# DJNing/articulated-object-nerf

Measured on AMD Instinct MI355X. Metric: rays/sec at 640×480×(64c+128f) samples; PSNR vs reference, higher is better.
Workload: dtype f16x3 (fp16 hi/lo split MFMA, fp32 accumulate)

## Files before the change

articulated-object-nerf_amd/aonerf/_lib.py:

```python
import ctypes
import os

import torch

_HERE = os.path.dirname(os.path.abspath(__file__))
LIB_PATH = os.path.join(os.path.dirname(_HERE), "lib", "libaonerf.so")

c_i64, c_int, c_float, c_size, vp = ctypes.c_int64, ctypes.c_int, ctypes.c_float, ctypes.c_size_t, ctypes.c_void_p

PREC = {"fp32": 0, "f16x3": 1}
PREC_F16X3_TRAIN = 1
PREC_BF16 = 2
ACT_NONE, ACT_VANILLA, ACT_ARTIC = 0, 1, 2
OPACITY = {None: 0, "mse": 1, "ce": 2, "autorf": 3}


class AonMlpParams(ctypes.Structure):
    _fields_ = [("pts_w", vp * 8), ("pts_b", vp * 8), ("density_w", vp), ("density_b", vp),
                ("bottleneck_w", vp), ("bottleneck_b", vp), ("views_w", vp), ("views_b", vp),
                ("rgb_w", vp), ("rgb_b", vp), ("w_rows", c_i64 * 12), ("w_cols", c_i64 * 12),
                ("b_len", c_i64 * 12)]


class AonMlpArtParams(ctypes.Structure):
    _fields_ = [("def_w", vp * 4), ("def_b", vp * 4), ("deformation_w", vp), ("deformation_b", vp),
                ("pts_w", vp * 8), ("pts_b", vp * 8), ("density_w", vp), ("density_b", vp),
# ... 336 lines not shown
```

articulated-object-nerf_amd/csrc/mlp.hip:

```cpp
#include "aon_common.hpp"
#include "mlp_layout.hpp"
#include "mlp_pipe.hpp"
#include "param_check.hpp"

namespace aon {
namespace mlp {

constexpr int kWaves = 8;
constexpr int kThreads = 64 * kWaves;
constexpr int kRowsPerWave = 16;
constexpr int kRowsPerBlock = kRowsPerWave * kWaves;

__device__ __forceinline__ f4 mfma(float a, float b, f4 c) {
  return __builtin_amdgcn_mfma_f32_16x16x4f32(a, b, c, 0, 0, 0);
}

template <int LAYER, int NA, int NB, int NACC>
__device__ __forceinline__ void gemm(Pipe<kThreads>& p, const f4 (&xa)[NA], const f4 (&xb)[NB],
                                     f4 (&acc)[NACC]) {
  constexpr LayerDesc d = kLayers[LAYER];
  constexpr int U = d.u;
  static_assert(U % 4 == 0 && U <= NACC && d.ka <= NA && d.kb <= NB, "layer/array mismatch");
#pragma unroll
  for (int t = 0; t < d.ka + d.kb; ++t) {
// ... 191 lines not shown
      while (li + 1 < kNumLayers && a.layers[li + 1].bias0 <= i) ++li;
      const int o = i - a.layers[li].bias0;
      if (o < a.layers[li].out_real) v = a.b[li][o];
    }
    out[e] = v;
  }
}

}
}

using namespace aon;
using namespace aon::mlp;

extern "C" size_t aon_mlp_packed_bytes(int precision) {
  if (precision == AON_PREC_FP32 || precision == AON_PREC_F16X3 || precision == AON_PREC_BF16)
    return kPackedBytesF32;
  return 0;
}

extern "C" int aon_mlp_read_status(const void* packed, size_t packed_bytes, uint32_t* status,
                                   aon_stream_t stream) {
  AON_REQUIRE(packed && status, "null pointer");
  AON_REQUIRE(packed_bytes >= kStatusBytes && packed_bytes % 16 == 0, "bad packed size");
  const char* word = static_cast<const char*>(packed) + packed_bytes - kStatusBytes;
  hipError_t e = hipMemcpyAsync(status, word, sizeof(uint32_t), hipMemcpyDeviceToHost,
                                (hipStream_t)stream);
  if (e == hipSuccess) e = hipStreamSynchronize((hipStream_t)stream);
  return static_cast<int>(e);
}

#ifndef AON_F16X3_NCOL
#define AON_F16X3_NCOL 1
#endif
static_assert(AON_F16X3_NCOL == 1 || AON_F16X3_NCOL == 2, "AON_F16X3_NCOL is 1 or 2");

extern "C" int aon_mlp_pack(const aon_mlp_params* prm, int precision, void* packed,
                            aon_stream_t stream) {
  AON_REQUIRE(prm && packed, "null pointer");
  AON_REQUIRE(precision == AON_PREC_FP32 || precision == AON_PREC_F16X3 ||
                  precision == AON_PREC_BF16,
              "unsupported precision");
  AON_REQUIRE(aligned16(packed), "packed buffer must be 16-byte aligned");
  if (check_mlp_params(prm, __func__)) return -1;
  PackArgs a;
  for (int i = 0; i < 8; ++i) {
    a.w[i] = prm->pts_w[i];
    a.b[i] = prm->pts_b[i];
  }
  a.w[LDEN] = prm->density_w;    a.b[LDEN] = prm->density_b;
  a.w[LBOT] = prm->bottleneck_w; a.b[LBOT] = prm->bottleneck_b;
  a.w[LVIEW] = prm->views_w;     a.b[LVIEW] = prm->views_b;
  a.w[LRGB] = prm->rgb_w;        a.b[LRGB] = prm->rgb_b;
  for (int i = 0; i < kNumLayers; ++i) {
    AON_REQUIRE(a.w[i] && a.b[i], "null layer parameter");
    a.layers[i] = precision == AON_PREC_FP32 ? kLayers[i] : kLayersH[i];
  }
  if (precision != AON_PREC_FP32)
    return pack_f16x3(a, packed, (hipStream_t)stream, precision == AON_PREC_BF16);
  const hipError_t e = hipMemsetAsync(static_cast<char*>(packed) + kPackedBytesF32 - kStatusBytes, 0,
                                      kStatusBytes, (hipStream_t)stream);
  if (e != hipSuccess) return static_cast<int>(e);
  const int64_t total = (int64_t)kStreamBlocks * 256 + kBiasFloats;
  hipLaunchKernelGGL(k_pack_f32, grid_for(total, 256, 4096), 256, 0, (hipStream_t)stream, a,
                     static_cast<float*>(packed));
  return launch_status(__func__);
}

static int mlp_launch(int mode, const void* packed, int precision, const float* a0,
                      const float* a1, const float* a2, const float* a3, int64_t B, int S,
                      int act, float* raw, aon_stream_t stream) {
  AON_REQUIRE(packed && raw && a0 && a1, "null pointer");
  AON_REQUIRE(precision == AON_PREC_FP32 || precision == AON_PREC_F16X3,
              "unsupported precision (AON_PREC_BF16 is the training forward's: aon_mlp_fwd_train_bf16)");
  AON_REQUIRE(B >= 0 && S >= 1, "bad shape");
  AON_REQUIRE(act >= AON_ACT_NONE && act <= AON_ACT_ARTIC, "bad activation");
  AON_REQUIRE(aligned16(packed) && aligned16(raw), "packed / raw must be 16-byte aligned");
  const int64_t N = B * S;
  if (N == 0) return 0;
  AON_REQUIRE((N + kRowsPerBlock - 1) / kRowsPerBlock < (1ll << 31), "too many rows");
#if AON_DATAFLOW_WS_BUILD
  if (precision == AON_PREC_F16X3 && mode == 0)
    return launch_ws_f16x3(packed, a0, a1, a2, a3, B, S, act, raw, (hipStream_t)stream);
#endif
  if (precision == AON_PREC_F16X3)
    return launch_f16x3(mode, AON_F16X3_NCOL, packed, a0, a1, a2, a3, B, S, act, raw,
                        (hipStream_t)stream);
// ... 64 lines not shown
```

articulated-object-nerf_amd/csrc/mlp_f16x3.hip:

```cpp
#include "mlp_f16x3_core.hpp"

namespace aon {
namespace mlp {

#ifndef AON_STASH_REGS
#define AON_STASH_REGS 0
#endif

#ifndef AON_STAGGER
#define AON_STAGGER 0
#endif

template <bool BF>
__host__ __device__ constexpr int stash_per() { return BF ? 3 : 6; }
template <bool BF>
__device__ __forceinline__ int enc_slot(int c, int k, int lo) { return BF ? 3 * c + k : 6 * c + 2 * k + lo; }
template <bool BF>
__device__ __forceinline__ int venc_slot(int c, int lo) { return BF ? 3 * c + 2 : 6 * c + 4 + lo; }

template <int NCOL, bool STORE, typename T, typename FP>
__device__ __forceinline__ void vanilla_layers(FP& fp, Frag<2, NCOL>& enc, Frag<1, NCOL>& venc,
                                               Frag<8, NCOL>& x, Frag<8, NCOL>& y, f4* stash,
                                               float* bias_s, int g, int wave,
                                               const int64_t (&rows)[NCOL], int64_t N, int act,
                                               float* __restrict__ raw, const TrainStore& ts) {
  constexpr bool BF = std::is_same<T, __bf16>::value;
  fp.start();
#if AON_PRIO_HALF
  if (wave >= GeomH<NCOL>::kWaves / 2) __builtin_amdgcn_s_setprio(AON_PRIO_HALF);
#endif
  lds_float* bias_l = opaque_lds(bias_s + 4 * g);

  Frag<1, NCOL> none;
  using SP = StorePick<STORE, NCOL, T>;
  T* const th = reinterpret_cast<T*>(ts.h);
  T* const tbot = reinterpret_cast<T*>(ts.bot);
  T* const thv = reinterpret_cast<T*>(ts.hv);
  const int64_t hs = act_rows(N) * 256;
  const int64_t ms = act_rows(N) * 4;
  layer_h<NetVanillaH, L0, true>(fp, none, enc, x, bias_l, g, SP::make(th, 256, rows, N, g, ts.masks));
  layer_h<NetVanillaH, L1, true>(fp, x, none, y, bias_l, g, SP::make(th + 1 * hs, 256, rows, N, g, ts.masks + 1 * ms));
  layer_h<NetVanillaH, L2, true>(fp, y, none, x, bias_l, g, SP::make(th + 2 * hs, 256, rows, N, g, ts.masks + 2 * ms));
  layer_h<NetVanillaH, L3, true>(fp, x, none, y, bias_l, g, SP::make(th + 3 * hs, 256, rows, N, g, ts.masks + 3 * ms));
  layer_h<NetVanillaH, L4, true>(fp, y, none, x, bias_l, g, SP::make(th + 4 * hs, 256, rows, N, g, ts.masks + 4 * ms));
#pragma unroll
  for (int c = 0; c < NCOL && !AON_STASH_REGS; ++c)
#pragma unroll
    for (int k = 0; k < 2; ++k) {
      enc.hi[k][c] = __builtin_bit_cast(h8, stash[64 * enc_slot<BF>(c, k, 0)]);
      if (!BF) enc.lo[k][c] = __builtin_bit_cast(h8, stash[64 * enc_slot<BF>(c, k, 1)]);
    }
  layer_h<NetVanillaH, L5, true>(fp, x, enc, y, bias_l, g, SP::make(th + 5 * hs, 256, rows, N, g, ts.masks + 5 * ms));
  layer_h<NetVanillaH, L6, true>(fp, y, none, x, bias_l, g, SP::make(th + 6 * hs, 256, rows, N, g, ts.masks + 6 * ms));
  layer_h<NetVanillaH, L7, true>(fp, x, none, y, bias_l, g, SP::make(th + 7 * hs, 256, rows, N, g, ts.masks + 7 * ms));
  f4 dens[NCOL], rgb[NCOL];
  head_h<NetVanillaH, LDEN>(fp, y, dens, bias_l, g);
  layer_h<NetVanillaH, LBOT, false>(fp, y, none, x, bias_l, g, SP::make(tbot, 256, rows, N, g));
#pragma unroll
  for (int c = 0; c < NCOL && !AON_STASH_REGS; ++c) {
    venc.hi[0][c] = __builtin_bit_cast(h8, stash[64 * venc_slot<BF>(c, 0)]);
    if (!BF) venc.lo[0][c] = __builtin_bit_cast(h8, stash[64 * venc_slot<BF>(c, 1)]);
  }
  layer_h<NetVanillaH, LVIEW, true>(fp, x, venc, y, bias_l, g, SP::make(thv, 128, rows, N, g, ts.masks + 8 * ms));
  head_h<NetVanillaH, LRGB>(fp, y, rgb, bias_l, g);

  if (g == 0) {
#pragma unroll
    for (int c = 0; c < NCOL; ++c) {
      if (rows[c] < N) {
        const float s = AON_F16X3_V2 ? 1.0f : 1.0f / kActScale;
        float sig = dens[c][0] * s;
        if (STORE && ts.noise) sig = __fadd_rn(sig, ts.noise[rows[c]]);
        const f4 o = {act_rgb(rgb[c][0] * s, act), act_rgb(rgb[c][1] * s, act),
                      act_rgb(rgb[c][2] * s, act), act_sigma(sig, act)};
#ifdef AON_ABL_NO_RAW_STORE
        if (__builtin_isnan(o[0] + o[1] + o[2] + o[3]))
#endif
        *reinterpret_cast<f4*>(raw + 4 * rows[c]) = o;
      }
    }
  }
}

template <int MODE, int NCOL, bool STORE = false, bool BF = false>
__global__ __launch_bounds__((GeomH<NCOL, BF>::kThreads), (GeomH<NCOL, BF>::kWavesPerSimd)) void k_mlp_fwd_f16x3(
    const f4* __restrict__ wstream, const float* __restrict__ bias_g, const float* __restrict__ in0,
    const float* __restrict__ in1, const float* __restrict__ in2, const float* __restrict__ in3,
    int64_t B, int S, int act, float* __restrict__ raw, TrainStore ts = {}) {
  using G = GeomH<NCOL, BF>;
  constexpr int kPer = stash_per<BF>() * NCOL;
  constexpr int kStash = AON_STASH_REGS ? 0 : G::kWaves * 64 * kPer;
  static_assert((kLdsWeights + kBiasFloats / 4 + kStash) * 16 <= 160 * 1024, "LDS");
  __shared__ f4 smem[kLdsWeights + kBiasFloats / 4 + kStash];
  float* bias_s = reinterpret_cast<float*>(smem + kLdsWeights);
  f4* stash = smem + kLdsWeights + kBiasFloats / 4 + (threadIdx.x >> 6) * 64 * kPer +
              (threadIdx.x & 63);

  const int tid = threadIdx.x, lane = tid & 63, wave = tid >> 6;
  const int g = lane >> 4, j = lane & 15;
  const int64_t N = B * S;

  WeightPipeP<NetVanillaH, G::kThreads, BF> p;
  p.wbuf = smem;
  p.src = wstream;
  p.tid = tid;
  p.lane = lane;
  p.start();
  for (int i = tid; i < kBiasFloats; i += G::kThreads) bias_s[i] = bias_g[i];

  Frag<2, NCOL> enc;
  Frag<1, NCOL> venc;
  int64_t rows[NCOL];
#pragma unroll
  for (int c = 0; c < NCOL; ++c) {
    const int64_t row = (int64_t)blockIdx.x * G::kRowsPerBlock + wave * G::kRowsPerWave + 16 * c + j;
    rows[c] = row;
    const int64_t rr = row < N ? row : N - 1;
    const int64_t ray = rr / S;
    float ev[2][8], vv[8];
    if (MODE == 0) {
      const float* ro = in0 + 3 * ray;
      const float* rd = in1 + 3 * ray;
      const float* vd = in2 + 3 * ray;
// ... 49 lines not shown
    split8<BF>(vv, venc.hi[0][c], venc.lo[0][c], venc.ovf);
  }

#pragma unroll
  for (int c = 0; c < NCOL && !AON_STASH_REGS; ++c) {
#pragma unroll
    for (int k = 0; k < 2; ++k) {
      stash[64 * enc_slot<BF>(c, k, 0)] = __builtin_bit_cast(f4, enc.hi[k][c]);
      if (!BF) stash[64 * enc_slot<BF>(c, k, 1)] = __builtin_bit_cast(f4, enc.lo[k][c]);
    }
    stash[64 * venc_slot<BF>(c, 0)] = __builtin_bit_cast(f4, venc.hi[0][c]);
    if (!BF) stash[64 * venc_slot<BF>(c, 1)] = __builtin_bit_cast(f4, venc.lo[0][c]);
  }

  Frag<8, NCOL> x, y;
  using WP = WeightPipeP<NetVanillaH, G::kThreads, BF>;
  using T = typename std::conditional<BF, __bf16, float>::type;
  if (AON_STAGGER && NCOL == 1 && !STORE && __builtin_amdgcn_readfirstlane(wave) >= G::kWaves / 2) {
    FragPipe<WP, AON_PREFETCH, 4, BF> fp(p);
    vanilla_layers<NCOL, STORE, T>(fp, enc, venc, x, y, stash, bias_s, g, wave, rows, N, act, raw, ts);
  } else {
    FragPipe<WP, AON_PREFETCH, 0, BF> fp(p);
    vanilla_layers<NCOL, STORE, T>(fp, enc, venc, x, y, stash, bias_s, g, wave, rows, N, act, raw, ts);
  }
  range_report(bias_g + kBiasFloats, ovf_of(x) | ovf_of(y) | enc.ovf | venc.ovf);
}

__global__ void k_pack_h(PackArgsH a, float* __restrict__ out_f) {
  const int64_t nhalf = (int64_t)a.stream_blocks * 512;
  _Float16* out = reinterpret_cast<_Float16*>(out_f);
  float* bias_out = out_f + (int64_t)a.stream_blocks * 256;
  const int64_t total = nhalf + a.bias_floats;
  const LayerDesc& last = a.layers[a.n_layers - 1];
  const int used_blocks = last.blk0 + (last.ka + last.kb) * last.u * 2;
  const StreamMap map{a.bf16, a.mx_lo, a.mx_hi};
  if (a.bf16 == 1 && !a.f16w && blockIdx.x == 0 && threadIdx.x < kStatusBytes / 4)
    reinterpret_cast<uint32_t*>(bias_out + a.bias_floats)[threadIdx.x] = 0u;
  for (int64_t e = blockIdx.x * (int64_t)blockDim.x + threadIdx.x; e < total;
       e += (int64_t)gridDim.x * blockDim.x) {
    if (e < nhalf) {
// ... 20 lines not shown
        const int o = 16 * u + (l & 15), gg = l >> 4;
        int col = -1;
        const float* src = a.w[li];
        int64_t ld = a.ldw[li];
        if (k < d.ka) {
          const int f = 32 * k + 16 * (jj >> 2) + 4 * gg + (jj & 3);
          col = f < d.len_a ? f : -1;
        } else {
          const int f = 32 * (k - d.ka) + 8 * gg + jj;
          col = f < d.len_b ? (a.w2[li] ? f : d.len_a + f) : -1;
          if (a.w2[li]) {
            src = a.w2[li];
            ld = a.ldw2[li];
          }
        }
        if (o < d.out_real && col >= 0)
          w = a.tr[li] ? src[(int64_t)col * ld + o] : src[(int64_t)o * ld + col];
      }
#if AON_F16X3_V2
      if (bf && !a.f16w) {
        out[e] = bf_bits(w);
        continue;
      }
      w *= kWS;
      const _Float16 h = static_cast<_Float16>(w);
      out[e] = lo_part ? static_cast<_Float16>(w - static_cast<float>(h)) : h;
      if (!lo_part && !(fabsf(w) <= kF16Max))
        *reinterpret_cast<uint32_t*>(bias_out + a.bias_floats) = 2u;
#else
      const _Float16 h = static_cast<_Float16>(w);
      out[e] = lo_part ? static_cast<_Float16>((w - static_cast<float>(h)) * kLoScale) : h;
#endif
    } else {
      const int i = static_cast<int>(e - nhalf);
      int li = 0;
      while (li + 1 < a.n_layers && a.layers[li + 1].bias0 <= i) ++li;
      const int o = i - a.layers[li].bias0;
#if AON_F16X3_V2
      const StreamMap map{a.bf16, a.mx_lo, a.mx_hi};
      const float bs =
          a.layers[li].u == 1 || !(map.f16(a.layers[li].blk0) || a.f16w) ? 1.0f : kActS;
#else
      const float bs = kActScale;
#endif
      bias_out[i] = (o < a.layers[li].out_real && a.b[li]) ? a.b[li][o] * bs : 0.f;
    }
  }
}

int pack_h(PackArgsH a, void* packed, hipStream_t stream) {
  const int64_t total = (int64_t)a.stream_blocks * 512 + a.bias_floats;
  if (a.bf16 != 1 || a.f16w) {
    const hipError_t e = hipMemsetAsync(
        static_cast<char*>(packed) + (size_t)a.stream_blocks * 1024 + (size_t)a.bias_floats * 4, 0,
        kStatusBytes, stream);
    if (e != hipSuccess) return static_cast<int>(e);
  }
  hipLaunchKernelGGL(k_pack_h, grid_for(total, 256, 4096), 256, 0, stream, a,
                     static_cast<float*>(packed));
  return launch_status("aon_mlp_pack");
}

int pack_f16x3(const PackArgs& a, void* packed, hipStream_t stream, bool bf16) {
  PackArgsH h{};
  h.bf16 = bf16 ? 1 : 0;
  for (int i = 0; i < kNumLayers; ++i) {
    h.w[i] = a.w[i];
    h.b[i] = a.b[i];
    h.layers[i] = kLayersH[i];
    h.ldw[i] = kLayersH[i].len_a + kLayersH[i].len_b;
  }
  h.n_layers = kNumLayers;
  h.stream_blocks = NetVanillaH::kStreamBlocks;
  h.bias_floats = NetVanillaH::kBiasFloats;
  return pack_h(h, packed, stream);
}

int launch_f16x3(int mode, int ncol, const void* packed, const float* a0, const float* a1,
                 const float* a2, const float* a3, int64_t B, int S, int act, float* raw,
                 hipStream_t stream, const TrainStore* ts) {
  const int64_t N = B * S;
  const f4* ws = static_cast<const f4*>(packed);
  const float* bias = reinterpret_cast<const float*>(static_cast<const char*>(packed) + kStreamBytesF32);
#define AON_LAUNCH_H(M, C)                                                                       \
  hipLaunchKernelGGL((k_mlp_fwd_f16x3<M, C>),                                                    \
                     static_cast<int>((N + GeomH<C>::kRowsPerBlock - 1) / GeomH<C>::kRowsPerBlock), \
                     GeomH<C>::kThreads, 0, stream, ws, bias, a0, a1, a2, a3, B, S, act, raw)
  if (mode == 2 || mode == 3) {
    const int grid = static_cast<int>((N + GeomH<1>::kRowsPerBlock - 1) / GeomH<1>::kRowsPerBlock);
    if (mode == 3) {
      using GB = GeomH<kBfNcolFwd, true>;
      hipLaunchKernelGGL((k_mlp_fwd_f16x3<0, kBfNcolFwd, true, true>),
                         static_cast<int>((N + GB::kRowsPerBlock - 1) / GB::kRowsPerBlock),
                         GB::kThreads, 0, stream, ws, bias, a0, a1, a2, a3, B, S, act, raw, *ts);
    } else
      hipLaunchKernelGGL((k_mlp_fwd_f16x3<0, 1, true>), grid, GeomH<1>::kThreads, 0, stream, ws,
                         bias, a0, a1, a2, a3, B, S, act, raw, *ts);
    return launch_status("aon_mlp_fwd_train");
  }
  if (mode == 0 && ncol == 1) AON_LAUNCH_H(0, 1);
  else if (mode == 0) AON_LAUNCH_H(0, 2);
  else if (ncol == 1) AON_LAUNCH_H(1, 1);
  else AON_LAUNCH_H(1, 2);
// ... 7 lines not shown
```

articulated-object-nerf_amd/csrc/mlp_layout.hpp:

```cpp
#pragma once

namespace aon {
namespace mlp {

struct LayerDesc {
  int ka, kb;
  int u;
  int len_a, len_b;
  int out_real;
  int blk0;
  int bias0;
};

enum { L0 = 0, L1, L2, L3, L4, L5, L6, L7, LDEN, LBOT, LVIEW, LRGB, kNumLayers };

constexpr int kChunk = 16;

constexpr LayerDesc kLayers[kNumLayers] = {
    {4, 0, 16, 63, 0, 256, 0, 0},
    {16, 0, 16, 256, 0, 256, 64, 256},
    {16, 0, 16, 256, 0, 256, 320, 512},
    {16, 0, 16, 256, 0, 256, 576, 768},
    {16, 0, 16, 256, 0, 256, 832, 1024},
    {16, 4, 16, 256, 63, 256, 1088, 1280},
// ... 7 lines not shown

constexpr LayerDesc kLayersH[kNumLayers] = {
    {0, 2, 16, 0, 63, 256, 0, 0},
    {8, 0, 16, 256, 0, 256, 64, 256},
    {8, 0, 16, 256, 0, 256, 320, 512},
    {8, 0, 16, 256, 0, 256, 576, 768},
    {8, 0, 16, 256, 0, 256, 832, 1024},
    {8, 2, 16, 256, 63, 256, 1088, 1280},
    {8, 0, 16, 256, 0, 256, 1408, 1536},
    {8, 0, 16, 256, 0, 256, 1664, 1792},
    {8, 0, 1, 256, 0, 1, 1920, 2048},
    {8, 0, 16, 256, 0, 256, 1936, 2064},
    {8, 1, 8, 256, 27, 128, 2192, 2320},
    {4, 0, 1, 128, 0, 3, 2336, 2448},
};

constexpr float kActScale = 1.0f / 256.0f;
constexpr float kLoScale = 2048.0f;
#ifndef AON_F16X3_V2
#define AON_F16X3_V2 1
#endif
constexpr float kActS = 8.0f;
constexpr float kWS = 64.0f;

constexpr int kBlocks = 2344;
constexpr int kStreamBlocks = (kBlocks + 63) / 64 * 64;
constexpr int kNumChunks = kStreamBlocks / kChunk;
constexpr int kBiasFloats = 2464;
constexpr size_t kStreamBytesF32 = (size_t)kStreamBlocks * 1024;
constexpr size_t kStatusBytes = 16;
// ... 111 lines not shown
    int blk = 0, bias = 0;
    for (int i = 0; i < NLAYERS; ++i) {
      const LayerDesc d = TABLE[i];
      if (d.blk0 != blk || d.bias0 != bias || d.blk0 % 2) return false;
      if (!(d.u == 1 || d.u % 2 == 0)) return false;
      if (d.len_a > 32 * d.ka || d.len_b > 32 * d.kb || d.out_real > 16 * d.u) return false;
      blk += (d.ka + d.kb) * d.u * 2;
      bias += d.u * 16;
    }
    return blk == BLOCKS && bias == BIAS_FLOATS && STREAM_BLOCKS >= BLOCKS &&
           STREAM_BLOCKS % 64 == 0;
  }
};

using NetVanillaH = NetH<kLayersH, kNumLayers, kBlocks, kStreamBlocks, kBiasFloats>;
using NetArtH = NetH<kLayersArt, kNumLayersArt, 2752, 2752, 3376>;
using NetBwdH = NetH<kLayersBwd, kNumLayersBwd, 2224, 2240, 2432, true>;
using NetArtBwdH = NetH<kLayersArtBwd, kNumLayersArtBwd, 2752, 2752, 3456, true>;
static_assert(NetVanillaH::ok(), "inconsistent vanilla fp16x3 layout");
static_assert(NetArtH::ok(), "inconsistent articulated fp16x3 layout");
static_assert(NetBwdH::ok(), "inconsistent backward-chain fp16x3 layout");
static_assert(NetArtBwdH::ok(), "inconsistent articulated backward-chain fp16x3 layout");

struct PackArgs {
  const float* w[kNumLayers];
  const float* b[kNumLayers];
  LayerDesc layers[kNumLayers];
};

constexpr int kMaxLayersH = 24;
struct PackArgsH {
  const float* w[kMaxLayersH];
  const float* w2[kMaxLayersH];
  const float* b[kMaxLayersH];
  int ldw[kMaxLayersH];
  int ldw2[kMaxLayersH];
  int tr[kMaxLayersH];
  LayerDesc layers[kMaxLayersH];
  int n_layers, stream_blocks, bias_floats;
  int bf16;
  int mx_lo, mx_hi;
  int f16w;
};

struct StreamMap {
  int mode, lo, hi;
  __host__ __device__ constexpr bool f16(int b) const {
    return mode == 0 || (mode == 2 && b >= lo && b < hi);
  }
  __host__ __device__ constexpr int map(int b) const {
    return mode == 0 ? b
         : mode == 1 ? b >> 1
         : b < lo    ? b >> 1
         : b < hi    ? (lo >> 1) + b - lo
                     : (lo >> 1) + (hi - lo) + ((b - hi) >> 1);
  }
  __host__ __device__ constexpr int unmap(int m) const {
// ... 32 lines not shown
  __bf16* enc_bf;
};

struct TrainStoreArt {
  float* hd;
  float* h;
  float* bot;
  float* hv;
  float* enc;
  float* xyz;
  const float* noise;
  uint2* masks;
  __bf16* enc_bf;
};

int pack_f16x3(const PackArgs& a, void* packed, hipStream_t stream, bool bf16 = false);
int pack_h(PackArgsH a, void* packed, hipStream_t stream);
int absmax(const float* x, int64_t n, uint32_t* out, hipStream_t stream);
int launch_f16x3(int mode, int ncol, const void* packed, const float* a0, const float* a1,
                 const float* a2, const float* a3, int64_t B, int S, int act, float* raw,
                 hipStream_t stream, const TrainStore* ts = nullptr);
#ifndef AON_DATAFLOW_WS_BUILD
#define AON_DATAFLOW_WS_BUILD 0
#endif
int launch_ws_f16x3(const void* packed, const float* a0, const float* a1, const float* a2,
                    const float* a3, int64_t B, int S, int act, float* raw, hipStream_t stream);
int launch_art_ws_f16x3(const void* packed, const float* a0, const float* a1, const float* a2,
                        const float* a3, int64_t B, int S, int act, float* raw, hipStream_t stream);

}
}
// ... 1 lines not shown
```

articulated-object-nerf_amd/csrc/mlp_ws.hip:

```cpp
#include <utility>

#include "mlp_f16x3_core.hpp"

namespace aon {
namespace mlp {
namespace ws {

#ifndef AON_WS_PREFETCH
#define AON_WS_PREFETCH 3
#endif

template <int WAVES>
struct Geo {
  static constexpr int kWaves = WAVES;
  static constexpr int kThreads = 64 * WAVES;
  static constexpr int kTiles = WAVES;
  static constexpr int kNb = 16 * kTiles;
  static constexpr int kActPlane = 8 * 4 * kNb;
  static constexpr int kEncPlane = 2 * 4 * kNb;
  static constexpr int kLdsF4 = 2 * kActPlane + 2 * kEncPlane;
  static constexpr int kWavesPerSimd = 2;
  static constexpr int kPrefetch = WAVES == 8 ? AON_WS_PREFETCH : AON_WS_PREFETCH - 1;
  static_assert(kLdsF4 * 16 * (8 / WAVES) <= 160 * 1024, "LDS");
  __host__ __device__ static constexpr int tu(int u) { return u / 2 >= WAVES ? u / WAVES : 2; }
// ... 244 lines not shown
  c.pl.act_hi = lds_base(smem + gj);
  c.pl.act_lo = lds_base(smem + G::kActPlane + gj);
  c.pl.enc_hi = lds_base(smem + 2 * G::kActPlane + gj);
  c.pl.enc_lo = lds_base(smem + 2 * G::kActPlane + G::kEncPlane + gj);
  c.row = (int64_t)blockIdx.x * G::kNb + 16 * c.w + c.j;
  c.rr = c.row < N ? c.row : N - 1;
  c.ray = c.rr / S;
  return c;
}

template <int WAVES>
__global__ __launch_bounds__(64 * WAVES, 2) void k_mlp_ws_f16x3(
    const f4* __restrict__ wstream, const float* __restrict__ bias_g, const float* __restrict__ in0,
    const float* __restrict__ in1, const float* __restrict__ in2, const float* __restrict__ in3,
    int64_t B, int S, int act, float* __restrict__ raw) {
  using Net = NetVanillaH;
  using G = Geo<WAVES>;
  __shared__ f4 smem[G::kLdsF4];
  const int64_t N = B * S;
  const WsSetup c = ws_setup<G>(smem, N, S);
  const int w = c.w, g = c.g;
  const Planes& pl = c.pl;
  APipe<Net, G, G::kPrefetch> ap;
  ap.ws = wstream;
  ap.lane = c.lane;
  ap.w = w;
  ap.start();

  uint64_t ovf = 0;
  {
    const float* ro = in0 + 3 * c.ray;
// ... 16 lines not shown
  hidden_layer<Net, G, L0, true>(ap, pl, bias_g, w, g, m16);
  hidden_layer<Net, G, L1, true>(ap, pl, bias_g, w, g, m16);
  hidden_layer<Net, G, L2, true>(ap, pl, bias_g, w, g, m16);
  hidden_layer<Net, G, L3, true>(ap, pl, bias_g, w, g, m16);
  hidden_layer<Net, G, L4, true>(ap, pl, bias_g, w, g, m16);
  hidden_layer<Net, G, L5, true>(ap, pl, bias_g, w, g, m16, [&] {
    const float* vd = in2 + 3 * c.ray;
    float vv[8];
#pragma unroll
    for (int e = 0; e < 8; ++e) vv[e] = pos_enc_feature(vd[0], vd[1], vd[2], 8 * g + e, 0, 4);
    put_segb<G>(pl, 0, w, vv, ovf);
  });
  hidden_layer<Net, G, L6, true>(ap, pl, bias_g, w, g, m16);
  hidden_layer<Net, G, L7, true>(ap, pl, bias_g, w, g, m16);
  const f4 dens = head<Net, G, LDEN>(ap, pl, bias_g, w, g);
  hidden_layer<Net, G, LBOT, false>(ap, pl, bias_g, w, g, m16);
  hidden_layer<Net, G, LVIEW, true>(ap, pl, bias_g, w, g, m16);
  const f4 rgb = head<Net, G, LRGB>(ap, pl, bias_g, w, g);
  if (g == 0 && c.row < N) {
    const f4 o = {act_rgb(rgb[0], act), act_rgb(rgb[1], act), act_rgb(rgb[2], act), act_sigma(dens[0], act)};
    *reinterpret_cast<f4*>(raw + 4 * c.row) = o;
  }
  const bool bad = (m16 & 0x7FFFu) >= 0x7C00u || ((m16 >> 16) & 0x7FFFu) >= 0x7C00u;
  range_report(bias_g + Net::kBiasFloats, ovf | __builtin_amdgcn_ballot_w64(bad));
}

template <int WAVES>
__global__ __launch_bounds__(64 * WAVES, 2) void k_mlp_art_ws_f16x3(
    const f4* __restrict__ wstream, const float* __restrict__ bias_g, const float* __restrict__ in0,
    const float* __restrict__ in1, const float* __restrict__ in2, const float* __restrict__ in3,
    int64_t B, int S, int act, float* __restrict__ raw) {
  using Net = NetArtH;
  using G = Geo<WAVES>;
// ... 311 lines not shown
#define AON_WS_HALVES(L_, RELU_, PREV, OUT)                                                  \
  f4 OUT##_a0[LG<Net, G, L_>::TU][LG<Net, G, L_>::NTh];                                     \
  half_mfma<Net, G, L_, 0>(ap, pl, w, OUT##_a0, PREV, m16);                                  \
  lds_barrier();                                                                             \
  const auto OUT##_j0 = make_job<Net, G, L_, RELU_, 0>(OUT##_a0, bias_g, w, g);              \
  f4 OUT##_a1[LG<Net, G, L_>::TU][LG<Net, G, L_>::NTh];                                     \
  half_mfma<Net, G, L_, 1>(ap, pl, w, OUT##_a1, OUT##_j0, m16);                              \
  lds_barrier();                                                                             \
  const auto OUT = make_job<Net, G, L_, RELU_, 1>(OUT##_a1, bias_g, w, g);

template <int WAVES>
__global__ __launch_bounds__(64 * WAVES, 2) void k_mlp_ws_pipe_f16x3(
    const f4* __restrict__ wstream, const float* __restrict__ bias_g, const float* __restrict__ in0,
    const float* __restrict__ in1, const float* __restrict__ in2, const float* __restrict__ in3,
    int64_t B, int S, int act, float* __restrict__ raw) {
  using Net = NetVanillaH;
  using G = Geo<WAVES>;
  __shared__ f4 smem[G::kLdsF4];
  const int64_t N = B * S;
  const WsSetup c = ws_setup<G>(smem, N, S);
  const int w = c.w, g = c.g;
  const Planes& pl = c.pl;
  APipeP<Net, G, G::kPrefetch> ap;
  ap.ws = wstream;
  ap.lane = c.lane;
  ap.w = w;
  ap.start();
  const bool first_half = w < G::kTiles / 2;

  uint64_t ovf = 0;
  {
// ... 20 lines not shown
  AON_WS_HALVES(L2, true, j1, j2)
  AON_WS_HALVES(L3, true, j2, j3)
  AON_WS_HALVES(L4, true, j3, j4)
  AON_WS_HALVES(L5, true, j4, j5)
  {
    const float* vd = in2 + 3 * c.ray;
    float vv[8];
#pragma unroll
    for (int e = 0; e < 8; ++e) vv[e] = pos_enc_feature(vd[0], vd[1], vd[2], 8 * g + e, 0, 4);
    put_segb<G>(pl, 0, w, vv, ovf);
  }
  AON_WS_HALVES(L6, true, j5, j6)
  AON_WS_HALVES(L7, true, j6, j7)
  f4 dens = {0.f, 0.f, 0.f, 0.f};
  if (first_half) dens = head_direct<Net, G, LDEN>(pl, wstream, bias_g, w, g, c.lane);
  f4 jb_a0[LG<Net, G, LBOT>::TU][LG<Net, G, LBOT>::NTh];
  half_mfma<Net, G, LBOT, 0>(ap, pl, w, jb_a0, j7, m16);
  lds_barrier();
  const auto jb_j0 = make_job<Net, G, LBOT, false, 0>(jb_a0, bias_g, w, g);
  if (!first_half) dens = head_direct<Net, G, LDEN>(pl, wstream, bias_g, w, g, c.lane);
  f4 jb_a1[LG<Net, G, LBOT>::TU][LG<Net, G, LBOT>::NTh];
  half_mfma<Net, G, LBOT, 1>(ap, pl, w, jb_a1, jb_j0, m16);
  lds_barrier();
  const auto jb = make_job<Net, G, LBOT, false, 1>(jb_a1, bias_g, w, g);
  AON_WS_HALVES(LVIEW, true, jb, jv)
  f4 rgb;
  if (first_half) rgb = head_direct<Net, G, LRGB>(pl, wstream, bias_g, w, g, c.lane);
  jv.all(pl, m16);
  lds_barrier();
  if (!first_half) rgb = head_direct<Net, G, LRGB>(pl, wstream, bias_g, w, g, c.lane);
  if (g == 0 && c.row < N) {
    const f4 o = {act_rgb(rgb[0], act), act_rgb(rgb[1], act), act_rgb(rgb[2], act), act_sigma(dens[0], act)};
    *reinterpret_cast<f4*>(raw + 4 * c.row) = o;
  }
  const bool bad = (m16 & 0x7FFFu) >= 0x7C00u || ((m16 >> 16) & 0x7FFFu) >= 0x7C00u;
  range_report(bias_g + Net::kBiasFloats, ovf | __builtin_amdgcn_ballot_w64(bad));
}
#undef AON_WS_HALVES

}

#ifndef AON_WS_PIPE
#define AON_WS_PIPE 0
#endif
static constexpr bool ws_pipe() { return AON_WS_PIPE == 1; }

#ifndef AON_WS_WAVES
#define AON_WS_WAVES 8
#endif
static constexpr int ws_waves() { return AON_WS_WAVES == 4 ? 4 : 8; }

int launch_ws_f16x3(const void* packed, const float* a0, const float* a1, const float* a2,
                    const float* a3, int64_t B, int S, int act, float* raw, hipStream_t stream) {
  const int64_t N = B * S;
  const f4* wsp = static_cast<const f4*>(packed);
  const float* bias = reinterpret_cast<const float*>(static_cast<const char*>(packed) + kStreamBytesF32);
  if (ws_pipe() && ws_waves() == 8)
    hipLaunchKernelGGL(ws::k_mlp_ws_pipe_f16x3<8>, static_cast<int>((N + 127) / 128), 512, 0,
                       stream, wsp, bias, a0, a1, a2, a3, B, S, act, raw);
  else if (ws_waves() == 8)
    hipLaunchKernelGGL(ws::k_mlp_ws_f16x3<8>, static_cast<int>((N + 127) / 128), 512, 0, stream,
                       wsp, bias, a0, a1, a2, a3, B, S, act, raw);
  else
    hipLaunchKernelGGL(ws::k_mlp_ws_f16x3<4>, static_cast<int>((N + 63) / 64), 256, 0, stream,
                       wsp, bias, a0, a1, a2, a3, B, S, act, raw);
  return launch_status("aon_mlp_fwd");
}

int launch_art_ws_f16x3(const void* packed, const float* a0, const float* a1, const float* a2,
                        const float* a3, int64_t B, int S, int act, float* raw, hipStream_t stream) {
  const int64_t N = B * S;
// ... 14 lines not shown
```

include/aonerf.h:

```cpp
#ifndef AONERF_H
#define AONERF_H

#include <stddef.h>
#include <stdint.h>

#ifdef __cplusplus
extern "C" {
#endif

typedef void* aon_stream_t;

#define AON_ABI_VERSION 13

#define AON_PREC_FP32 0
#define AON_PREC_F16X3 1
#define AON_PREC_BF16 2

#define AON_ACT_NONE 0
#define AON_ACT_VANILLA 1
#define AON_ACT_ARTIC 2

int aon_abi_version(void);
const char* aon_last_error(void);

int aon_ray_directions(int H, int W, float focal, float* dirs, aon_stream_t stream);

int aon_get_rays(const float* dirs, int64_t n, const float* c2w_host, float* rays_o,
                 float* rays_d, float* viewdirs, int H, int W, float* radii,
                 aon_stream_t stream);

// ... 247 lines not shown
```

Before: 1.405 million.

## Fold the linear bottleneck layer into the view layer for f16x3 inference

Because the bottleneck layer has no activation, its weights and bias are multiplied into the views layer's feature-input weights and bias at pack time, in double precision. The inference kernels (both the streaming and warp-specialized variants) skip one 256x256 GEMM and stream fewer weight blocks. A separate F16X3_TRAIN precision keeps the unfolded layout for training, since training needs the bottleneck activation. The folded weights are rounded to the fp16 hi/lo split once, which may change numerics slightly.

```diff
diff --git a/articulated-object-nerf_amd/aonerf/_lib.py b/articulated-object-nerf_amd/aonerf/_lib.py
--- a/articulated-object-nerf_amd/aonerf/_lib.py
+++ b/articulated-object-nerf_amd/aonerf/_lib.py
@@ -9,7 +9,7 @@
 c_i64, c_int, c_float, c_size, vp = ctypes.c_int64, ctypes.c_int, ctypes.c_float, ctypes.c_size_t, ctypes.c_void_p
 
 PREC = {"fp32": 0, "f16x3": 1}
-PREC_F16X3_TRAIN = 1
+PREC_F16X3_TRAIN = 4
 PREC_BF16 = 2
 ACT_NONE, ACT_VANILLA, ACT_ARTIC = 0, 1, 2
 OPACITY = {None: 0, "mse": 1, "ce": 2, "autorf": 3}
diff --git a/articulated-object-nerf_amd/csrc/mlp.hip b/articulated-object-nerf_amd/csrc/mlp.hip
--- a/articulated-object-nerf_amd/csrc/mlp.hip
+++ b/articulated-object-nerf_amd/csrc/mlp.hip
@@ -229,7 +229,8 @@
 using namespace aon::mlp;
 
 extern "C" size_t aon_mlp_packed_bytes(int precision) {
-  if (precision == AON_PREC_FP32 || precision == AON_PREC_F16X3 || precision == AON_PREC_BF16)
+  if (precision == AON_PREC_F16X3) return NetVanillaFoldH::kPackedBytes;
+  if (precision == AON_PREC_FP32 || precision == AON_PREC_F16X3_TRAIN || precision == AON_PREC_BF16)
     return kPackedBytesF32;
   return 0;
 }
@@ -254,7 +255,7 @@
                             aon_stream_t stream) {
   AON_REQUIRE(prm && packed, "null pointer");
   AON_REQUIRE(precision == AON_PREC_FP32 || precision == AON_PREC_F16X3 ||
-                  precision == AON_PREC_BF16,
+                  precision == AON_PREC_F16X3_TRAIN || precision == AON_PREC_BF16,
               "unsupported precision");
   AON_REQUIRE(aligned16(packed), "packed buffer must be 16-byte aligned");
   if (check_mlp_params(prm, __func__)) return -1;
@@ -272,7 +273,8 @@
     a.layers[i] = precision == AON_PREC_FP32 ? kLayers[i] : kLayersH[i];
   }
   if (precision != AON_PREC_FP32)
-    return pack_f16x3(a, packed, (hipStream_t)stream, precision == AON_PREC_BF16);
+    return pack_f16x3(a, packed, (hipStream_t)stream, precision == AON_PREC_BF16,
+                      precision == AON_PREC_F16X3);
   const hipError_t e = hipMemsetAsync(static_cast<char*>(packed) + kPackedBytesF32 - kStatusBytes, 0,
                                       kStatusBytes, (hipStream_t)stream);
   if (e != hipSuccess) return static_cast<int>(e);
@@ -286,6 +288,9 @@
                       const float* a1, const float* a2, const float* a3, int64_t B, int S,
                       int act, float* raw, aon_stream_t stream) {
   AON_REQUIRE(packed && raw && a0 && a1, "null pointer");
+  AON_REQUIRE(precision != AON_PREC_F16X3_TRAIN,
+              "AON_PREC_F16X3_TRAIN is the training forward's stream (aon_mlp_fwd_train): render "
+              "with an AON_PREC_F16X3 pack");
   AON_REQUIRE(precision == AON_PREC_FP32 || precision == AON_PREC_F16X3,
               "unsupported precision (AON_PREC_BF16 is the training forward's: aon_mlp_fwd_train_bf16)");
   AON_REQUIRE(B >= 0 && S >= 1, "bad shape");
diff --git a/articulated-object-nerf_amd/csrc/mlp_f16x3.hip b/articulated-object-nerf_amd/csrc/mlp_f16x3.hip
--- a/articulated-object-nerf_amd/csrc/mlp_f16x3.hip
+++ b/articulated-object-nerf_amd/csrc/mlp_f16x3.hip
@@ -18,7 +18,7 @@
 template <bool BF>
 __device__ __forceinline__ int venc_slot(int c, int lo) { return BF ? 3 * c + 2 : 6 * c + 4 + lo; }
 
-template <int NCOL, bool STORE, typename T, typename FP>
+template <typename Net, int NCOL, bool STORE, typename T, typename FP>
 __device__ __forceinline__ void vanilla_layers(FP& fp, Frag<2, NCOL>& enc, Frag<1, NCOL>& venc,
                                                Frag<8, NCOL>& x, Frag<8, NCOL>& y, f4* stash,
                                                float* bias_s, int g, int wave,
@@ -38,11 +38,11 @@
   T* const thv = reinterpret_cast<T*>(ts.hv);
   const int64_t hs = act_rows(N) * 256;
   const int64_t ms = act_rows(N) * 4;
-  layer_h<NetVanillaH, L0, true>(fp, none, enc, x, bias_l, g, SP::make(th, 256, rows, N, g, ts.masks));
-  layer_h<NetVanillaH, L1, true>(fp, x, none, y, bias_l, g, SP::make(th + 1 * hs, 256, rows, N, g, ts.masks + 1 * ms));
-  layer_h<NetVanillaH, L2, true>(fp, y, none, x, bias_l, g, SP::make(th + 2 * hs, 256, rows, N, g, ts.masks + 2 * ms));
-  layer_h<NetVanillaH, L3, true>(fp, x, none, y, bias_l, g, SP::make(th + 3 * hs, 256, rows, N, g, ts.masks + 3 * ms));
-  layer_h<NetVanillaH, L4, true>(fp, y, none, x, bias_l, g, SP::make(th + 4 * hs, 256, rows, N, g, ts.masks + 4 * ms));
+  layer_h<Net, L0, true>(fp, none, enc, x, bias_l, g, SP::make(th, 256, rows, N, g, ts.masks));
+  layer_h<Net, L1, true>(fp, x, none, y, bias_l, g, SP::make(th + 1 * hs, 256, rows, N, g, ts.masks + 1 * ms));
+  layer_h<Net, L2, true>(fp, y, none, x, bias_l, g, SP::make(th + 2 * hs, 256, rows, N, g, ts.masks + 2 * ms));
+  layer_h<Net, L3, true>(fp, x, none, y, bias_l, g, SP::make(th + 3 * hs, 256, rows, N, g, ts.masks + 3 * ms));
+  layer_h<Net, L4, true>(fp, y, none, x, bias_l, g, SP::make(th + 4 * hs, 256, rows, N, g, ts.masks + 4 * ms));
 #pragma unroll
   for (int c = 0; c < NCOL && !AON_STASH_REGS; ++c)
 #pragma unroll
@@ -50,19 +50,27 @@
       enc.hi[k][c] = __builtin_bit_cast(h8, stash[64 * enc_slot<BF>(c, k, 0)]);
       if (!BF) enc.lo[k][c] = __builtin_bit_cast(h8, stash[64 * enc_slot<BF>(c, k, 1)]);
     }
-  layer_h<NetVanillaH, L5, true>(fp, x, enc, y, bias_l, g, SP::make(th + 5 * hs, 256, rows, N, g, ts.masks + 5 * ms));
-  layer_h<NetVanillaH, L6, true>(fp, y, none, x, bias_l, g, SP::make(th + 6 * hs, 256, rows, N, g, ts.masks + 6 * ms));
-  layer_h<NetVanillaH, L7, true>(fp, x, none, y, bias_l, g, SP::make(th + 7 * hs, 256, rows, N, g, ts.masks + 7 * ms));
+  layer_h<Net, L5, true>(fp, x, enc, y, bias_l, g, SP::make(th + 5 * hs, 256, rows, N, g, ts.masks + 5 * ms));
+  layer_h<Net, L6, true>(fp, y, none, x, bias_l, g, SP::make(th + 6 * hs, 256, rows, N, g, ts.masks + 6 * ms));
+  layer_h<Net, L7, true>(fp, x, none, y, bias_l, g, SP::make(th + 7 * hs, 256, rows, N, g, ts.masks + 7 * ms));
   f4 dens[NCOL], rgb[NCOL];
-  head_h<NetVanillaH, LDEN>(fp, y, dens, bias_l, g);
-  layer_h<NetVanillaH, LBOT, false>(fp, y, none, x, bias_l, g, SP::make(tbot, 256, rows, N, g));
+  head_h<Net, LDEN>(fp, y, dens, bias_l, g);
+  constexpr bool FOLD = std::is_same<Net, NetVanillaFoldH>::value;
+  static_assert(!FOLD || !STORE, "the training forwards keep the bottleneck activation");
+  if constexpr (!FOLD)
+    layer_h<Net, LBOT, false>(fp, y, none, x, bias_l, g, SP::make(tbot, 256, rows, N, g));
 #pragma unroll
   for (int c = 0; c < NCOL && !AON_STASH_REGS; ++c) {
     venc.hi[0][c] = __builtin_bit_cast(h8, stash[64 * venc_slot<BF>(c, 0)]);
     if (!BF) venc.lo[0][c] = __builtin_bit_cast(h8, stash[64 * venc_slot<BF>(c, 1)]);
   }
-  layer_h<NetVanillaH, LVIEW, true>(fp, x, venc, y, bias_l, g, SP::make(thv, 128, rows, N, g, ts.masks + 8 * ms));
-  head_h<NetVanillaH, LRGB>(fp, y, rgb, bias_l, g);
+  if constexpr (FOLD) {
+    layer_h<Net, LF_VIEW, true>(fp, y, venc, x, bias_l, g);
+    head_h<Net, LF_RGB>(fp, x, rgb, bias_l, g);
+  } else {
+    layer_h<Net, LVIEW, true>(fp, x, venc, y, bias_l, g, SP::make(thv, 128, rows, N, g, ts.masks + 8 * ms));
+    head_h<Net, LRGB>(fp, y, rgb, bias_l, g);
+  }
 
   if (g == 0) {
 #pragma unroll
@@ -82,7 +90,7 @@
   }
 }
 
-template <int MODE, int NCOL, bool STORE = false, bool BF = false>
+template <int MODE, int NCOL, bool STORE = false, bool BF = false, typename Net = NetVanillaH>
 __global__ __launch_bounds__((GeomH<NCOL, BF>::kThreads), (GeomH<NCOL, BF>::kWavesPerSimd)) void k_mlp_fwd_f16x3(
     const f4* __restrict__ wstream, const float* __restrict__ bias_g, const float* __restrict__ in0,
     const float* __restrict__ in1, const float* __restrict__ in2, const float* __restrict__ in3,
@@ -90,23 +98,23 @@
   using G = GeomH<NCOL, BF>;
   constexpr int kPer = stash_per<BF>() * NCOL;
   constexpr int kStash = AON_STASH_REGS ? 0 : G::kWaves * 64 * kPer;
-  static_assert((kLdsWeights + kBiasFloats / 4 + kStash) * 16 <= 160 * 1024, "LDS");
-  __shared__ f4 smem[kLdsWeights + kBiasFloats / 4 + kStash];
+  static_assert((kLdsWeights + Net::kBiasFloats / 4 + kStash) * 16 <= 160 * 1024, "LDS");
+  __shared__ f4 smem[kLdsWeights + Net::kBiasFloats / 4 + kStash];
   float* bias_s = reinterpret_cast<float*>(smem + kLdsWeights);
-  f4* stash = smem + kLdsWeights + kBiasFloats / 4 + (threadIdx.x >> 6) * 64 * kPer +
+  f4* stash = smem + kLdsWeights + Net::kBiasFloats / 4 + (threadIdx.x >> 6) * 64 * kPer +
               (threadIdx.x & 63);
 
   const int tid = threadIdx.x, lane = tid & 63, wave = tid >> 6;
   const int g = lane >> 4, j = lane & 15;
   const int64_t N = B * S;
 
-  WeightPipeP<NetVanillaH, G::kThreads, BF> p;
+  WeightPipeP<Net, G::kThreads, BF> p;
   p.wbuf = smem;
   p.src = wstream;
   p.tid = tid;
   p.lane = lane;
   p.start();
-  for (int i = tid; i < kBiasFloats; i += G::kThreads) bias_s[i] = bias_g[i];
+  for (int i = tid; i < Net::kBiasFloats; i += G::kThreads) bias_s[i] = bias_g[i];
 
   Frag<2, NCOL> enc;
   Frag<1, NCOL> venc;
@@ -186,16 +194,16 @@
   }
 
   Frag<8, NCOL> x, y;
-  using WP = WeightPipeP<NetVanillaH, G::kThreads, BF>;
+  using WP = WeightPipeP<Net, G::kThreads, BF>;
   using T = typename std::conditional<BF, __bf16, float>::type;
   if (AON_STAGGER && NCOL == 1 && !STORE && __builtin_amdgcn_readfirstlane(wave) >= G::kWaves / 2) {
     FragPipe<WP, AON_PREFETCH, 4, BF> fp(p);
-    vanilla_layers<NCOL, STORE, T>(fp, enc, venc, x, y, stash, bias_s, g, wave, rows, N, act, raw, ts);
+    vanilla_layers<Net, NCOL, STORE, T>(fp, enc, venc, x, y, stash, bias_s, g, wave, rows, N, act, raw, ts);
   } else {
     FragPipe<WP, AON_PREFETCH, 0, BF> fp(p);
-    vanilla_layers<NCOL, STORE, T>(fp, enc, venc, x, y, stash, bias_s, g, wave, rows, N, act, raw, ts);
-  }
-  range_report(bias_g + kBiasFloats, ovf_of(x) | ovf_of(y) | enc.ovf | venc.ovf);
+    vanilla_layers<Net, NCOL, STORE, T>(fp, enc, venc, x, y, stash, bias_s, g, wave, rows, N, act, raw, ts);
+  }
+  range_report(bias_g + Net::kBiasFloats, ovf_of(x) | ovf_of(y) | enc.ovf | venc.ovf);
 }
 
 __global__ void k_pack_h(PackArgsH a, float* __restrict__ out_f) {
@@ -246,8 +254,17 @@
             ld = a.ldw2[li];
           }
         }
-        if (o < d.out_real && col >= 0)
-          w = a.tr[li] ? src[(int64_t)col * ld + o] : src[(int64_t)o * ld + col];
+        if (o < d.out_real && col >= 0) {
+          if (a.fold_w && li == a.fold_layer && k < d.ka) {
+            double acc = 0.0;
+            for (int j = 0; j < a.fold_k; ++j)
+              acc = fma(static_cast<double>(src[(int64_t)o * ld + j]),
+                        static_cast<double>(a.fold_w[(int64_t)j * d.len_a + col]), acc);
+            w = static_cast<float>(acc);
+          } else {
+            w = a.tr[li] ? src[(int64_t)col * ld + o] : src[(int64_t)o * ld + col];
+          }
+        }
       }
 #if AON_F16X3_V2
       if (bf && !a.f16w) {
@@ -275,7 +292,15 @@
 #else
       const float bs = kActScale;
 #endif
-      bias_out[i] = (o < a.layers[li].out_real && a.b[li]) ? a.b[li][o] * bs : 0.f;
+      float b = (o < a.layers[li].out_real && a.b[li]) ? a.b[li][o] : 0.f;
+      if (a.fold_w && li == a.fold_layer && o < a.layers[li].out_real) {
+        double acc = 0.0;
+        for (int j = 0; j < a.fold_k; ++j)
+          acc = fma(static_cast<double>(a.w[li][(int64_t)o * a.ldw[li] + j]),
+                    static_cast<double>(a.fold_b[j]), acc);
+        b = static_cast<float>(static_cast<double>(b) + acc);
+      }
+      bias_out[i] = b * bs;
     }
   }
 }
@@ -293,9 +318,26 @@
   return launch_status("aon_mlp_pack");
 }
 
-int pack_f16x3(const PackArgs& a, void* packed, hipStream_t stream, bool bf16) {
+int pack_f16x3(const PackArgs& a, void* packed, hipStream_t stream, bool bf16, bool fold) {
   PackArgsH h{};
   h.bf16 = bf16 ? 1 : 0;
+  if (fold) {
+    for (int i = 0; i < kNumLayersFold; ++i) {
+      const int src = i < LBOT ? i : i + 1;
+      h.w[i] = a.w[src];
+      h.b[i] = a.b[src];
+      h.layers[i] = kLayersHFold[i];
+      h.ldw[i] = kLayersHFold[i].len_a + kLayersHFold[i].len_b;
+    }
+    h.fold_w = a.w[LBOT];
+    h.fold_b = a.b[LBOT];
+    h.fold_layer = LF_VIEW;
+    h.fold_k = kLayersH[LBOT].out_real;
+    h.n_layers = kNumLayersFold;
+    h.stream_blocks = NetVanillaFoldH::kStreamBlocks;
+    h.bias_floats = NetVanillaFoldH::kBiasFloats;
+    return pack_h(h, packed, stream);
+  }
   for (int i = 0; i < kNumLayers; ++i) {
     h.w[i] = a.w[i];
     h.b[i] = a.b[i];
@@ -313,12 +355,15 @@
                  hipStream_t stream, const TrainStore* ts) {
   const int64_t N = B * S;
   const f4* ws = static_cast<const f4*>(packed);
-  const float* bias = reinterpret_cast<const float*>(static_cast<const char*>(packed) + kStreamBytesF32);
+  const bool train = mode == 2 || mode == 3;
+  const float* bias = reinterpret_cast<const float*>(
+      static_cast<const char*>(packed) +
+      (train ? NetVanillaH::kStreamBytes : NetVanillaFoldH::kStreamBytes));
 #define AON_LAUNCH_H(M, C)                                                                       \
-  hipLaunchKernelGGL((k_mlp_fwd_f16x3<M, C>),                                                    \
+  hipLaunchKernelGGL((k_mlp_fwd_f16x3<M, C, false, false, NetVanillaFoldH>),                     \
                      static_cast<int>((N + GeomH<C>::kRowsPerBlock - 1) / GeomH<C>::kRowsPerBlock), \
                      GeomH<C>::kThreads, 0, stream, ws, bias, a0, a1, a2, a3, B, S, act, raw)
-  if (mode == 2 || mode == 3) {
+  if (train) {
     const int grid = static_cast<int>((N + GeomH<1>::kRowsPerBlock - 1) / GeomH<1>::kRowsPerBlock);
     if (mode == 3) {
       using GB = GeomH<kBfNcolFwd, true>;
diff --git a/articulated-object-nerf_amd/csrc/mlp_layout.hpp b/articulated-object-nerf_amd/csrc/mlp_layout.hpp
--- a/articulated-object-nerf_amd/csrc/mlp_layout.hpp
+++ b/articulated-object-nerf_amd/csrc/mlp_layout.hpp
@@ -45,6 +45,25 @@
     {8, 1, 8, 256, 27, 128, 2192, 2320},
     {4, 0, 1, 128, 0, 3, 2336, 2448},
 };
+
+enum { LF_VIEW = LDEN + 1, LF_RGB, kNumLayersFold };
+
+constexpr LayerDesc kLayersHFold[kNumLayersFold] = {
+    {0, 2, 16, 0, 63, 256, 0, 0},
+    {8, 0, 16, 256, 0, 256, 64, 256},
+    {8, 0, 16, 256, 0, 256, 320, 512},
+    {8, 0, 16, 256, 0, 256, 576, 768},
+    {8, 0, 16, 256, 0, 256, 832, 1024},
+    {8, 2, 16, 256, 63, 256, 1088, 1280},
+    {8, 0, 16, 256, 0, 256, 1408, 1536},
+    {8, 0, 16, 256, 0, 256, 1664, 1792},
+    {8, 0, 1, 256, 0, 1, 1920, 2048},
+    {8, 1, 8, 256, 27, 128, 1936, 2064},
+    {4, 0, 1, 128, 0, 3, 2080, 2192},
+};
+constexpr int kBlocksFold = 2088;
+constexpr int kStreamBlocksFold = (kBlocksFold + 63) / 64 * 64;
+constexpr int kBiasFloatsFold = 2208;
 
 constexpr float kActScale = 1.0f / 256.0f;
 constexpr float kLoScale = 2048.0f;
@@ -186,10 +205,27 @@
 };
 
 using NetVanillaH = NetH<kLayersH, kNumLayers, kBlocks, kStreamBlocks, kBiasFloats>;
+using NetVanillaFoldH =
+    NetH<kLayersHFold, kNumLayersFold, kBlocksFold, kStreamBlocksFold, kBiasFloatsFold>;
 using NetArtH = NetH<kLayersArt, kNumLayersArt, 2752, 2752, 3376>;
 using NetBwdH = NetH<kLayersBwd, kNumLayersBwd, 2224, 2240, 2432, true>;
 using NetArtBwdH = NetH<kLayersArtBwd, kNumLayersArtBwd, 2752, 2752, 3456, true>;
 static_assert(NetVanillaH::ok(), "inconsistent vanilla fp16x3 layout");
+static_assert(NetVanillaFoldH::ok(), "inconsistent folded vanilla fp16x3 layout");
+constexpr bool layout_fold_ok() {
+  for (int i = 0; i < kNumLayersFold; ++i) {
+    const LayerDesc& f = kLayersHFold[i];
+    const LayerDesc& h = kLayersH[i < LBOT ? i : i + 1];
+    if (f.ka != h.ka || f.kb != h.kb || f.u != h.u || f.len_a != h.len_a || f.len_b != h.len_b ||
+        f.out_real != h.out_real)
+      return false;
+    if (i < LBOT && (f.blk0 != h.blk0 || f.bias0 != h.bias0)) return false;
+  }
+  const LayerDesc& b = kLayersH[LBOT];
+  return kLayersHFold[LF_VIEW].len_a == b.out_real && kBlocksFold == kBlocks - b.ka * b.u * 2 &&
+         kBiasFloatsFold == kBiasFloats - b.u * 16;
+}
+static_assert(layout_fold_ok(), "folded layout must be kLayersH without the bottleneck");
 static_assert(NetArtH::ok(), "inconsistent articulated fp16x3 layout");
 static_assert(NetBwdH::ok(), "inconsistent backward-chain fp16x3 layout");
 static_assert(NetArtBwdH::ok(), "inconsistent articulated backward-chain fp16x3 layout");
@@ -213,6 +249,9 @@
   int bf16;
   int mx_lo, mx_hi;
   int f16w;
+  const float* fold_w;
+  const float* fold_b;
+  int fold_layer, fold_k;
 };
 
 struct StreamMap {
@@ -275,7 +314,8 @@
   __bf16* enc_bf;
 };
 
-int pack_f16x3(const PackArgs& a, void* packed, hipStream_t stream, bool bf16 = false);
+int pack_f16x3(const PackArgs& a, void* packed, hipStream_t stream, bool bf16 = false,
+               bool fold = false);
 int pack_h(PackArgsH a, void* packed, hipStream_t stream);
 int absmax(const float* x, int64_t n, uint32_t* out, hipStream_t stream);
 int launch_f16x3(int mode, int ncol, const void* packed, const float* a0, const float* a1,
diff --git a/articulated-object-nerf_amd/csrc/mlp_ws.hip b/articulated-object-nerf_amd/csrc/mlp_ws.hip
--- a/articulated-object-nerf_amd/csrc/mlp_ws.hip
+++ b/articulated-object-nerf_amd/csrc/mlp_ws.hip
@@ -282,7 +282,7 @@
     const f4* __restrict__ wstream, const float* __restrict__ bias_g, const float* __restrict__ in0,
     const float* __restrict__ in1, const float* __restrict__ in2, const float* __restrict__ in3,
     int64_t B, int S, int act, float* __restrict__ raw) {
-  using Net = NetVanillaH;
+  using Net = NetVanillaFoldH;
   using G = Geo<WAVES>;
   __shared__ f4 smem[G::kLdsF4];
   const int64_t N = B * S;
@@ -329,9 +329,8 @@
   hidden_layer<Net, G, L6, true>(ap, pl, bias_g, w, g, m16);
   hidden_layer<Net, G, L7, true>(ap, pl, bias_g, w, g, m16);
   const f4 dens = head<Net, G, LDEN>(ap, pl, bias_g, w, g);
-  hidden_layer<Net, G, LBOT, false>(ap, pl, bias_g, w, g, m16);
-  hidden_layer<Net, G, LVIEW, true>(ap, pl, bias_g, w, g, m16);
-  const f4 rgb = head<Net, G, LRGB>(ap, pl, bias_g, w, g);
+  hidden_layer<Net, G, LF_VIEW, true>(ap, pl, bias_g, w, g, m16);
+  const f4 rgb = head<Net, G, LF_RGB>(ap, pl, bias_g, w, g);
   if (g == 0 && c.row < N) {
     const f4 o = {act_rgb(rgb[0], act), act_rgb(rgb[1], act), act_rgb(rgb[2], act), act_sigma(dens[0], act)};
     *reinterpret_cast<f4*>(raw + 4 * c.row) = o;
@@ -673,7 +672,7 @@
     const f4* __restrict__ wstream, const float* __restrict__ bias_g, const float* __restrict__ in0,
     const float* __restrict__ in1, const float* __restrict__ in2, const float* __restrict__ in3,
     int64_t B, int S, int act, float* __restrict__ raw) {
-  using Net = NetVanillaH;
+  using Net = NetVanillaFoldH;
   using G = Geo<WAVES>;
   __shared__ f4 smem[G::kLdsF4];
   const int64_t N = B * S;
@@ -724,21 +723,20 @@
   AON_WS_HALVES(L7, true, j6, j7)
   f4 dens = {0.f, 0.f, 0.f, 0.f};
   if (first_half) dens = head_direct<Net, G, LDEN>(pl, wstream, bias_g, w, g, c.lane);
-  f4 jb_a0[LG<Net, G, LBOT>::TU][LG<Net, G, LBOT>::NTh];
-  half_mfma<Net, G, LBOT, 0>(ap, pl, w, jb_a0, j7, m16);
+  f4 jv_a0[LG<Net, G, LF_VIEW>::TU][LG<Net, G, LF_VIEW>::NTh];
+  half_mfma<Net, G, LF_VIEW, 0>(ap, pl, w, jv_a0, j7, m16);
   lds_barrier();
-  const auto jb_j0 = make_job<Net, G, LBOT, false, 0>(jb_a0, bias_g, w, g);
+  const auto jv_j0 = make_job<Net, G, LF_VIEW, true, 0>(jv_a0, bias_g, w, g);
   if (!first_half) dens = head_direct<Net, G, LDEN>(pl, wstream, bias_g, w, g, c.lane);
-  f4 jb_a1[LG<Net, G, LBOT>::TU][LG<Net, G, LBOT>::NTh];
-  half_mfma<Net, G, LBOT, 1>(ap, pl, w, jb_a1, jb_j0, m16);
+  f4 jv_a1[LG<Net, G, LF_VIEW>::TU][LG<Net, G, LF_VIEW>::NTh];
+  half_mfma<Net, G, LF_VIEW, 1>(ap, pl, w, jv_a1, jv_j0, m16);
   lds_barrier();
-  const auto jb = make_job<Net, G, LBOT, false, 1>(jb_a1, bias_g, w, g);
-  AON_WS_HALVES(LVIEW, true, jb, jv)
+  const auto jv = make_job<Net, G, LF_VIEW, true, 1>(jv_a1, bias_g, w, g);
   f4 rgb;
-  if (first_half) rgb = head_direct<Net, G, LRGB>(pl, wstream, bias_g, w, g, c.lane);
+  if (first_half) rgb = head_direct<Net, G, LF_RGB>(pl, wstream, bias_g, w, g, c.lane);
   jv.all(pl, m16);
   lds_barrier();
-  if (!first_half) rgb = head_direct<Net, G, LRGB>(pl, wstream, bias_g, w, g, c.lane);
+  if (!first_half) rgb = head_direct<Net, G, LF_RGB>(pl, wstream, bias_g, w, g, c.lane);
   if (g == 0 && c.row < N) {
     const f4 o = {act_rgb(rgb[0], act), act_rgb(rgb[1], act), act_rgb(rgb[2], act), act_sigma(dens[0], act)};
     *reinterpret_cast<f4*>(raw + 4 * c.row) = o;
@@ -764,7 +762,8 @@
                     const float* a3, int64_t B, int S, int act, float* raw, hipStream_t stream) {
   const int64_t N = B * S;
   const f4* wsp = static_cast<const f4*>(packed);
-  const float* bias = reinterpret_cast<const float*>(static_cast<const char*>(packed) + kStreamBytesF32);
+  const float* bias = reinterpret_cast<const float*>(static_cast<const char*>(packed) +
+                                                    NetVanillaFoldH::kStreamBytes);
   if (ws_pipe() && ws_waves() == 8)
     hipLaunchKernelGGL(ws::k_mlp_ws_pipe_f16x3<8>, static_cast<int>((N + 127) / 128), 512, 0,
                        stream, wsp, bias, a0, a1, a2, a3, B, S, act, raw);
diff --git a/include/aonerf.h b/include/aonerf.h
--- a/include/aonerf.h
+++ b/include/aonerf.h
@@ -14,6 +14,7 @@
 
 #define AON_PREC_FP32 0
 #define AON_PREC_F16X3 1
+#define AON_PREC_F16X3_TRAIN 4
 #define AON_PREC_BF16 2
 
 #define AON_ACT_NONE 0
```

Result: faster. 1.568 million (median of 6 runs) (+11.6%).
